# anneouyang/OuterSPACE

Hardware: AMD Instinct MI355X
Metric: spgemm_output_nnz_per_s (higher is better)
Workload: dtype f64

## Files before the change

### outerspace_amd/csrc/osp_api.hip

```cpp
#include <hip/hip_runtime.h>

#include <algorithm>
#include <cmath>
#include <cstdarg>
#include <cstdio>
#include <cstdlib>
#include <chrono>
#include <cstring>
#include <functional>
#include <limits>
#include <map>
#include <memory>
#include <string>
#include <vector>

#include "../../include/outerspace_spgemm.h"
#include "../../include/outerspace_spgemm_masked.h"
#include "../../include/outerspace_spgemm_mcl.h"
#include "../../include/outerspace_spgemm_apply_mask.h"
#include "../../include/outerspace_spgemm_select.h"
#include "../../include/outerspace_spgemm_ewise.h"
#include "../../include/outerspace_spgemm_vector.h"
#include "../../include/outerspace_spgemm_mxm.h"
#include "../../include/outerspace_spgemm_transpose.h"
// ... 193 lines not shown
    uint64_t P = 0;
    const int algo = cfg.algorithm;
    if (algo != OSP_ALGO_OUTER && algo != OSP_ALGO_ROWWISE) throw Error(OSP_ERR_ARG, "unknown algorithm");
    const bool rowwise = algo == OSP_ALGO_ROWWISE && nnz && (uint64_t)nnz_b < 0xffffffffull && nnz < 0xffffffffull && !partials_only;
    ChunkTable<T> ct{};
    const uint64_t direct_min_nnz = getenv("OSP_DIRECT_MIN_NNZ") ? strtoull(getenv("OSP_DIRECT_MIN_NNZ"), nullptr, 10) : ((getenv("OSP_GATHER") && atoi(getenv("OSP_GATHER")) == 0) ? (8ull << 20) : (2ull << 20));
    const bool dense_avg = (long double)p_all * 8.0L >= 3.0L * (long double)M * (long double)N;
    const bool direct = nnz && (nnz >= direct_min_nnz || dense_avg) && (uint64_t)nnz_b < 0xffffffffull && nnz < 0xffffffffull && !partials_only &&
                        !(getenv("OSP_DIRECT") && atoi(getenv("OSP_DIRECT")) == 0);
    const uint64_t direct_max = std::min<uint64_t>(getenv("OSP_DIRECT_MAX") ? strtoull(getenv("OSP_DIRECT_MAX"), nullptr, 10) : kSplitRowMax,
                                                   kDirectDenseMax);
    const int gather_env = getenv("OSP_GATHER") ? atoi(getenv("OSP_GATHER")) : 2;
    const bool gather_ok = nnz && !rowwise && !partials_only && (uint64_t)nnz_b < 0xffffffffull && nnz < 0xffffffffull;
    const bool gather_short = gather_ok && gather_env >= 2 && direct;
    ShortRuns<T> srun{};
    DirectSrc dsrc{};
    uint32_t n_long_rows = 1;
    if (nnz == 0) {
        OSP_HIP(hipMemsetAsync(row_off, 0, (M + 1) * sizeof(uint64_t), s));
    } else {
        Scratch ss(ctx);
        Scratch &keep = (rowwise || direct || gather_short) ? sc : ss;
        const RowSort rs(ss, nnz, std::max(1, bits_for(M)));
        uint32_t *rows_sorted = (gather_short ? keep : ss).template get<uint32_t>(nnz), *perm = keep.get<uint32_t>(nnz), *w_sorted = ss.get<uint32_t>(nnz);
        uint32_t *bs_sorted = (rowwise || direct || gather_short) ? keep.get<uint32_t>(nnz) : nullptr;
        uint32_t *rowfirst = keep.get<uint32_t>(M + 1);
        uint64_t *offs_sorted = keep.get<uint64_t>(nnz + 1);
        uint64_t *scan_tmp = ss.get<uint64_t>(scan_scratch_entries(std::max<uint64_t>(nnz, M + 1)));
        const bool table = rowwise || direct || gather_short;
        const bool with_av = gather_ok && gather_env >= 1 && (direct || gather_short);
        T *av_sorted = with_av ? keep.get<T>(nnz) : nullptr;
        uint32_t *w = ss.get<uint32_t>(with_av ? 4 * nnz : table ? 2 * nnz : nnz);
        uint32_t *bs = table ? w : nullptr;
        sym_chunk_len_kernel<<<grid_for(nnz, 256), 256, 0, s>>>(a_colptr, b_rowptr, k0, k1, e0, nnz, w, bs,
                                                                with_av ? reinterpret_cast<const uint32_t *>(a_vals) : nullptr, (uint32_t)(sizeof(T) / 4));
        SymEpilogue sym_ep{w, bs, rows_sorted, perm, w_sorted, bs_sorted};
        if (with_av) { sym_ep.av_sorted = av_sorted; sym_ep.vwords = (uint32_t)(sizeof(T) / 4); }
        rs.sort(a_rowidx + e0, sym_ep);
        device_exclusive_scan<LoadU32As64, uint64_t>(LoadU32As64{w_sorted}, nnz, offs_sorted, scan_tmp, s);
        sym_row_offsets_kernel<<<grid_for(M + 1, 256), 256, 0, s>>>(rows_sorted, offs_sorted, nnz, M, row_off, rowfirst);
        const uint64_t rw_cap = (rowwise || gather_short) ? (uint64_t)TileCap<T>::value : 0ull;
        const bool expand_rows_on = gather_short && !(getenv("OSP_EXPAND_ROWS") && atoi(getenv("OSP_EXPAND_ROWS")) == 0);
        if (!expand_rows_on) sym_scatter_offsets_kernel<<<grid_for(nnz, 256), 256, 0, s>>>(perm, offs_sorted, rows_sorted, row_off, rw_cap, nnz, chunk_off);
        if (partials_only || rowwise || row_sharded) P = d2h(offs_sorted + nnz, s);
        else P = kPartialsOnDevice;
        if (direct) {
            dsrc = DirectSrc{rowfirst, offs_sorted, bs_sorted, perm, b_colidx, chunk_off, direct_max};
            dsrc.b_rowptr = b_rowptr; dsrc.K = K; dsrc.nnz_b = (uint64_t)nnz_b; dsrc.keep = &sc;
            dsrc.gather = gather_ok && gather_env >= 1;
            dsrc.expand_rows = expand_rows_on;
            if (expand_rows_on) { dsrc.chunk_off_ready = false; dsrc.rows_sorted = rows_sorted; dsrc.row_off = row_off; dsrc.rw_cap = rw_cap; dsrc.nnz = nnz; }
            dsrc.a_vals = with_av ? (const void *)av_sorted : (const void *)(a_vals + e0); dsrc.av_in_order = with_av; dsrc.b_vals = b_vals;
            if (dsrc.gather) {
                dsrc.gstat = (unsigned long long *)sc.get<uint64_t>(3);
                zero_async(s, {{dsrc.gstat, 3 * sizeof(uint64_t)}});
            }
        }
        if (gather_short) {
            const ShortRunFlag sf{offs_sorted};
            uint32_t *cidx = ss.get<uint32_t>(nnz + 1), *cidx_tmp = ss.get<uint32_t>(scan_scratch_entries(nnz + 1));
            device_exclusive_scan<ShortRunFlag, uint32_t>(sf, nnz, cidx, cidx_tmp, s);
            RunDesc<T> *runs0 = sc.get<RunDesc<T>>(nnz);
            uint32_t *rowfirst0 = sc.get<uint32_t>(M + 1);
            short_runs_kernel<T><<<grid_for(nnz, 256), 256, 0, s>>>(sf, cidx, nnz, bs_sorted, av_sorted, runs0);
            short_rowfirst_kernel<<<grid_for(M + 1, 256), 256, 0, s>>>(rowfirst, cidx, M, rowfirst0);
            srun = ShortRuns<T>{runs0, rowfirst0, b_colidx, b_vals};
        }
        if (rowwise) {
            ct = ChunkTable<T>{offs_sorted, bs_sorted, perm, rowfirst, a_vals + e0, b_colidx, b_vals, (uint32_t)rw_cap, 1u};
            uint32_t *flag_scan = ss.get<uint32_t>(M + 1);
            device_exclusive_scan<HeavyRowFlag, uint32_t>(HeavyRowFlag{row_off, 0, (uint32_t)rw_cap}, M, flag_scan, (uint32_t *)scan_tmp, s);
            n_long_rows = d2h(flag_scan + M, s);
        }
    }
    tm.end(PH_SYM);
    res->info.partials = P;

    OuterProducer<T> prod;
    prod.ctx = ctx; prod.res = res;
    prod.a_colptr = a_colptr; prod.a_rowidx = a_rowidx; prod.a_vals = a_vals;
    prod.b_rowptr = b_rowptr; prod.b_colidx = b_colidx; prod.b_vals = b_vals;
    prod.k0 = k0; prod.k1 = k1; prod.e0 = e0; prod.chunk_off = chunk_off;
    const uint64_t nk = k1 - k0;
    prod.a_start = sc.get<int64_t>(nk); prod.a_cnt = sc.get<uint32_t>(nk);
    prod.prod = sc.get<uint64_t>(nk); prod.prod_off = sc.get<uint64_t>(nk + 1);
    prod.scan_tmp = sc.get<uint64_t>(scan_scratch_entries(nk));
    prod.nothing_staged = rowwise && n_long_rows == 0;
    prod.short_gathered = gather_short;
    if ((dsrc.gather || gather_short) && nnz && !partials_only) {
        prod.nnz = nnz;
        prod.kscan = sc.get<uint32_t>(nnz + 1);
        prod.kscan_tmp = sc.get<uint32_t>(scan_scratch_entries(std::max<uint64_t>(nnz, k1 - k0) + 1));
        prod.elist = sc.get<uint32_t>(nnz);
        prod.cscan = sc.get<uint32_t>(k1 - k0 + 1);
        prod.klist = sc.get<uint32_t>(k1 - k0 + 1);
    }

    if (partials_only) {
        if (row_sharded) throw Error(OSP_ERR_ARG, "partial products of a row shard are not supported");
        res->partials = true;
        res->rowptr = (int64_t *)ctx->alloc((M + 1) * sizeof(int64_t));
        OSP_HIP(hipMemcpyAsync(res->rowptr, row_off, (M + 1) * sizeof(uint64_t), hipMemcpyDeviceToDevice, s));
        res->vals = ctx->alloc(std::max<uint64_t>(P, 1) * sizeof(Part<T>));
        res->info.panels = 1;
        res->info.nnz_c = P;
        res->info.row_begin = 0;
        res->info.row_end = M;
        tm.begin(PH_MUL);
        if (P) prod.produce(0, M, true, 0, P, (Part<T> *)res->vals, tm, nullptr, nullptr);
        tm.end(PH_MUL);
        finish_timing(res, ev, tm, s);
        return;
    }
    const uint64_t off_lo = 0, P_rows = P;
    merge_pipeline<T>(ctx, res, prod, M, N, row_off, P_rows, cfg.partial_capacity, tm, r_lo, r_hi, off_lo, sink,
                      rowwise ? &ct : nullptr, (direct && nnz) ? &dsrc : nullptr, nullptr, gather_short ? &srun : nullptr);

    finish_timing(res, ev, tm, s);
    if (gather_short) res->info.gathered_short_partials = res->info.partials - res->info.heavy_partials;
    if (dsrc.gstat && res->info.direct_rows) {
        uint64_t gs[3] = {0, 0, 0};
        copy_d2h(gs, dsrc.gstat, sizeof(gs), s);
        res->info.gathered_rows = gs[0]; res->info.gathered_partials = gs[1]; res->info.gathered_runs = gs[2];
    }
    if (getenv("OSP_VERBOSE")) {
        fprintf(stderr, "[osp] product done in %.1f ms; pool misses so far: %llu hipMalloc calls, %.1f GB, %.1f ms\n", res->info.ms_total,
                (unsigned long long)ctx->malloc_calls, ctx->malloc_bytes / 1e9, ctx->malloc_ms);
    }
}

template <class T>
static void coo_to_compressed_device(Context *ctx, Scratch &sc, uint64_t nseg, uint64_t ninner, uint64_t nnz, const uint32_t *seg,
                                     const uint32_t *inner, const T *vals, const char *what, int64_t **ptr_out,
                                     uint32_t **idx_out, T **val_out) {
    hipStream_t s = ctx->stream;
    int64_t *ptr = sc.get<int64_t>(nseg + 1);
    uint32_t *idx = sc.get<uint32_t>(nnz);
    T *ov = sc.get<T>(nnz);
    *ptr_out = ptr; *idx_out = idx; *val_out = ov;
    if (nnz == 0) {
        OSP_HIP(hipMemsetAsync(ptr, 0, (nseg + 1) * sizeof(int64_t), s));
        return;
    }
    Scratch ss(ctx);
    uint32_t *flags = ss.get<uint32_t>(1);
    OSP_HIP(hipMemsetAsync(flags, 0, sizeof(uint32_t), s));
    const CooOrder o = coo_sort_two_keys(ss, nnz, inner, std::max(1, bits_for(ninner)), seg, std::max(1, bits_for(nseg)));
    ingest_finish_kernel<T><<<grid_for(nnz, 256), 256, 0, s>>>(o.outer_sorted, o.perm, inner, vals, nnz, nseg, ninner, idx, ov, flags);
    ingest_ptr_kernel<<<grid_for(nseg + 1, 256), 256, 0, s>>>(o.outer_sorted, nnz, nseg, ptr);
    check_flags(d2h(flags, s), what);
}

template <class T>
static void spgemm_coo_impl(Context *ctx, Result *res, uint64_t M, uint64_t K, uint64_t N, uint64_t nnz_a, const uint32_t *a_rows,
                            const uint32_t *a_cols, const T *a_vals, uint64_t nnz_b, const uint32_t *b_rows, const uint32_t *b_cols,
                            const T *b_vals, osp_memspace_t space, const osp_config_t &cfg) {
    hipStream_t s = ctx->stream;
    Scratch sc(ctx);
    EventPair ev;
    OSP_HIP(hipEventRecord(ev.a, s));
    const uint32_t *ar = to_device(sc, a_rows, nnz_a, space, s), *ac = to_device(sc, a_cols, nnz_a, space, s);
    const uint32_t *br = to_device(sc, b_rows, nnz_b, space, s), *bc = to_device(sc, b_cols, nnz_b, space, s);
    const T *av = to_device(sc, a_vals, nnz_a, space, s), *bv = to_device(sc, b_vals, nnz_b, space, s);
    int64_t *ap, *bp;
    uint32_t *ai, *bi;
    T *acv, *bcv;
    coo_to_compressed_device<T>(ctx, sc, K, M, nnz_a, ac, ar, av, "A (COO)", &ap, &ai, &acv);
    coo_to_compressed_device<T>(ctx, sc, K, N, nnz_b, br, bc, bv, "B (COO)", &bp, &bi, &bcv);
    OSP_HIP(hipEventRecord(ev.b, s));
    osp_config_t c2 = cfg;
    c2.validate = 0;
    spgemm_impl<T>(ctx, res, M, K, N, ap, ai, acv, bp, bi, bcv, OSP_DEVICE, c2);
    const float ms = ev.ms();
    res->info.ms_ingest = ms;
    res->info.ms_total += ms;
}
// ... 993 lines not shown
```

### outerspace_amd/csrc/osp_pipeline.h

```cpp
#pragma once

#define OSP_WITH_RA(ctx_, ...)                                               \
    do {                                                                     \
        if ((ctx_)->rank_atomic) { constexpr bool RA = true; __VA_ARGS__; }  \
        else { constexpr bool RA = false; __VA_ARGS__; }                     \
    } while (0)

template <class T> struct Producer {
    virtual ~Producer() {}
    virtual void produce(uint64_t r0, uint64_t r1, bool whole, uint64_t base, uint64_t count,
                         Part<T> *stage, PhaseTimer &tm, const uint32_t *cells = nullptr, Part<T> *qstage = nullptr,
                         const HubArgs *hub = nullptr, bool compact = false, bool has_long = true, bool desc_only = false, bool walk_all = false) = 0;
};

template <class T> struct MergeIO {
    Part<T> *stage;
    const uint64_t *row_off; uint64_t r0, r1, base;
    int64_t *c_rowptr; uint32_t *c_col; T *c_val;
    const uint64_t *out_in; uint64_t *out_out;
    ChunkTable<T> ct{};
    uint32_t *abort_word = nullptr;
    const RunDesc<T> *runs0 = nullptr; const uint32_t *rowfirst0 = nullptr; const uint32_t *b_colidx = nullptr; const T *b_vals = nullptr;
};
template <class T> struct ShortRuns {
// ... 164 lines not shown
        device_exclusive_scan<LoadU64, uint64_t>(LoadU64{nhist}, nlong, pl.hbase, pl.hscan_tmp, s);
        if (ds) device_exclusive_scan<LoadU64, uint64_t>(LoadU64{ncellh}, nlong, pl.cellbase, pl.hscan_tmp, s);
        if (ds && nrund) device_exclusive_scan<LoadU64, uint64_t>(LoadU64{nrund}, nlong, rdbase, pl.hscan_tmp, s);
        ndcell = 0;
        nrd = 0;
        {
            Gather g(s);
            g.add(&pl.nh, (const uint64_t *)pl.hoff + nlong); g.add(&pl.nblocks, (const uint64_t *)pl.blkbase + nlong);
            g.add(&pl.nvirt, (const uint64_t *)pl.vbase + nlong); g.add(&pl.ncell, (const uint64_t *)pl.hbase + nlong);
            if (ds) g.add(&ndcell, (const uint64_t *)pl.cellbase + nlong);
            if (ds && nrund) g.add(&nrd, (const uint64_t *)rdbase + nlong);
            for (int i = 0; i < 6; i++) g.add(&tot[i], (const uint64_t *)totals + i);
            g.add(&nsmall, (const uint64_t *)totals + 6);
            g.wait();
        }
        if (ds && ndcell >= 0xffffffffull) { ds = nullptr; hub_b = 0; continue; }
        if (hub_possible && !hub_decided && hub_b == 0 && pl.nblocks && (double)tot[3 + kModeStretch] >= hub_min_share * (double)count) {
            hub_decided = true;
            hub_b = hub_b_want;
            continue;
        }
        break;
    }
    for (int m = 0; m < 3; m++) { pl.mode_rows[m] = tot[m]; pl.mode_partials[m] = tot[3 + m]; }
    if (pl.nh >= 0xffffffffull) throw Error(OSP_ERR_CAPACITY, "long rows of one panel exceed 2^32 partial products");
    res->info.heavy_rows += nlong;
    res->info.heavy_partials += pl.nh;
    res->info.direct_rows += pl.mode_rows[kModeDirect];
    res->info.direct_partials += pl.mode_partials[kModeDirect];
    if (pl.ncell >= 0xffffffffull || pl.nblocks >= 0x7fffffffull || pl.nvirt >= 0xffffffffull || ndcell >= 0xffffffffull)
        throw Error(OSP_ERR_CAPACITY, "split histogram too large");
    if (getenv("OSP_VERBOSE"))
        fprintf(stderr, "[osp]   panel rows [%llu,%llu): %u tiles, %u long rows with %llu partial products -> %llu segments; direct: %llu rows, %llu "
                        "partial products, %llu cells\n",
                (unsigned long long)r0, (unsigned long long)r1, pl.p0.ntiles, nlong, (unsigned long long)pl.nh, (unsigned long long)pl.nvirt,
                (unsigned long long)pl.mode_rows[kModeDirect], (unsigned long long)pl.mode_partials[kModeDirect], (unsigned long long)ndcell);
    pl.ghist = sc.get<uint32_t>(pl.ncell + 1);
    pl.ghist_tmp = sc.get<uint32_t>(scan_scratch_entries(pl.ncell + 1));
    pl.vrow_off = sc.get<uint64_t>(pl.nvirt + 1);
    pl.vfirst = sc.get<uint8_t>(pl.nvirt + 1);
    pl.vcol0 = sc.get<uint32_t>(pl.nvirt + 1);
    pl.vcol1 = sc.get<uint32_t>(pl.nvirt + 1);
    if (pl.mode_rows[kModeDirect]) {
        pl.cells = sc.get<uint32_t>(ndcell);
        GatherPlan gp{};
        RunDesc<T> *runs = nullptr;
        static const uint64_t max_runs = getenv("OSP_GATHER_MAX_RUNS") ? strtoull(getenv("OSP_GATHER_MAX_RUNS"), nullptr, 10) : 0xffffffffull;
        if (ds->gather && nrund && nrd < max_runs) {
            runs = sc.get<RunDesc<T>>(std::max<uint64_t>(nrd, 1));
            pl.vrun_off = sc.get<uint32_t>(pl.nvirt + 1);
            pl.vrun_end = sc.get<uint32_t>(pl.nvirt + 1);
            gp.rdbase = rdbase; gp.vrun_off = pl.vrun_off; gp.vrun_end = pl.vrun_end;
            gp.rowruns = sc.get<uint32_t>(nlong);
            pl.nwritten = gp.nwritten = sc.get<uint32_t>(1);
            fill_async(s, {{pl.vrun_off, (pl.nvirt + 1) * sizeof(uint32_t), kNoRuns}, {gp.rowruns, (uint64_t)nlong * sizeof(uint32_t), kNoRuns},
                           {pl.nwritten, sizeof(uint32_t), 0u}});
            gp.over = !(getenv("OSP_GATHER_OVER") && atoi(getenv("OSP_GATHER_OVER")) == 0);
            gp.av_in_order = ds->av_in_order ? 1u : 0u;
            pl.may_write = !gp.over;
            pl.ga.runs = runs; pl.ga.b_colidx = ds->b_colidx; pl.ga.b_vals = (const T *)ds->b_vals;
        }
        if (!(runs && gp.over) || (hub_b && pl.nblocks)) ds->ensure_chunk_off(s);
        gp.mark_skipped = ds->chunk_off_ready ? 1u : 0u;
        const bool plan_small = runs != nullptr && gp.over && nsmall != 0;
        const bool plan_big = !plan_small || nsmall < pl.mode_rows[kModeDirect];
        if (plan_small) gp.small = hsmall;
        if (getenv("OSP_VERBOSE"))
            fprintf(stderr, "[osp]   small planner: %llu of %llu direct rows (at most %u chunks, %u cells)\n", (unsigned long long)(plan_small ? nsmall : 0),
                    (unsigned long long)pl.mode_rows[kModeDirect], small_lim.chunks, small_lim.cells);
        tm.begin(PH_PLAN_K, s);
        if (plan_small)
            direct_plan_small_kernel<T><<<nlong, kWave, direct_plan_small_lds(small_lim.cells), s>>>(
                pl.p0.long_rows, nlong, pl.hbits, nseg, pl.vbase, pl.hoff, colbits, kCap, ds->rowfirst, ds->off, ds->bs, ds->perm, ds->b_colidx,
                pl.vrow_off, pl.vcol0, pl.vcol1, ds->chunk_off, gp, (const T *)ds->a_vals, runs);
        if (!plan_big) {  }
        else if (nlong <= 4u * ctx->cus)
            direct_plan_kernel<T, kDirectCellsBig><<<nlong, kDirectThreads, 0, s>>>(pl.p0.long_rows, nlong, pl.hmode, pl.hbits, nseg, pl.vbase, pl.hoff,
                                                                                 pl.cellbase, row_off, colbits, kCap, ds->rowfirst, ds->off, ds->bs, ds->perm,
                                                                                 ds->b_colidx, pl.vrow_off, pl.vcol0, pl.vcol1, pl.cells, ds->chunk_off, gp,
                                                                                 (const T *)ds->a_vals, runs);
        else
        direct_plan_kernel<T><<<nlong, kDirectThreads, 0, s>>>(pl.p0.long_rows, nlong, pl.hmode, pl.hbits, nseg, pl.vbase, pl.hoff, pl.cellbase, row_off,
                                                              colbits, kCap, ds->rowfirst, ds->off, ds->bs, ds->perm, ds->b_colidx, pl.vrow_off,
                                                              pl.vcol0, pl.vcol1, pl.cells, ds->chunk_off, gp, (const T *)ds->a_vals, runs);
        tm.end(PH_PLAN_K);
        if (gp.rowruns && ds->gstat) gather_stats_kernel<<<std::min(grid_for(nlong, 256), 64u), 256, 0, s>>>(pl.p0.long_rows, nlong, row_off, gp.rowruns, ds->gstat);
#ifdef OSP_PLAN_PROF
        if (getenv("OSP_VERBOSE")) {
            unsigned long long hp[8] = {0}, z[8] = {0};
            OSP_HIP(hipStreamSynchronize(s));
            (void)hipMemcpyFromSymbol(hp, HIP_SYMBOL(osp_plan_prof), sizeof(hp));
            (void)hipMemcpyToSymbol(HIP_SYMBOL(osp_plan_prof), z, sizeof(z));
            double tot = 0;
            for (int k = 0; k < 6; k++) tot += (double)hp[k];
            fprintf(stderr, "[osp]   planner cycles: header %.1f %%, chunk descriptors %.1f %%, histogram pass %.1f %%, grouping %.1f %%, cell pass %.1f %%, "
                            "prefixes + output %.1f %%; %.0f cycles per row, %u rows\n", 100 * hp[0] / tot, 100 * hp[1] / tot, 100 * hp[2] / tot, 100 * hp[3] / tot,
                    100 * hp[4] / tot, 100 * hp[5] / tot, tot / std::max(1u, nlong), nlong);
            (void)hipMemcpyFromSymbol(hp, HIP_SYMBOL(osp_plan_small_prof), sizeof(hp));
            (void)hipMemcpyToSymbol(HIP_SYMBOL(osp_plan_small_prof), z, sizeof(z));
            tot = 0;
            for (int k = 0; k < 5; k++) tot += (double)hp[k];
            if (plan_small && tot > 0)
                fprintf(stderr, "[osp]   small planner cycles: header + chunk descriptors %.1f %%, histogram pass %.1f %%, grouping %.1f %%, counts %.1f %%, "
                                "prefixes + output %.1f %%; %.0f cycles per row, %llu rows\n", 100 * hp[0] / tot, 100 * hp[1] / tot, 100 * hp[2] / tot,
                        100 * hp[3] / tot, 100 * hp[4] / tot, tot / (double)nsmall, (unsigned long long)nsmall);
        }
#endif
        res->info.direct_plan_launches++;
        dbg_sync(s, "plan of the direct rows");
    }
    if (hub_b && pl.nblocks) {
        if (!ds->hub.sx) {
            Scratch &keep = *ds->keep;
            const uint64_t nb = ds->nnz_b;
            Scratch tmp(ctx);
            uint8_t *rowstart = tmp.get<uint8_t>(nb + 4);
            uint32_t *sx = keep.get<uint32_t>(nb + 1), *runstart = keep.get<uint32_t>(nb + 1);
            uint16_t *runblk = keep.get<uint16_t>(nb + 2);
            uint32_t *scan_tmp = tmp.get<uint32_t>(scan_scratch_entries(nb + 1));
            OSP_HIP(hipMemsetAsync(rowstart, 0, nb + 4, s));
            hub_rowstart_kernel<<<grid_for(ds->K, 256), 256, 0, s>>>(ds->b_rowptr, ds->K, rowstart);
            const int sh = colbits - hub_b;
            const HubRunFlag flag{rowstart, ds->b_colidx, sh};
            device_exclusive_scan<HubRunFlag, uint32_t>(flag, nb, sx, scan_tmp, s);
            compact_flagged_kernel<HubRunFlag><<<grid_for(nb, 256), 256, 0, s>>>(flag, sx, nb, 0, runstart);
            hub_runstart_end_kernel<<<1, 1, 0, s>>>(sx + nb, runstart, (uint32_t)nb);
            OSP_HIP(hipMemsetAsync(runblk, 0, (nb + 2) * sizeof(uint16_t), s));
            hub_runblk_kernel<<<std::min(grid_for(nb, 256), 4096u), 256, 0, s>>>(sx + nb, runstart, ds->b_colidx, sh, runblk);
            OSP_HIP(hipStreamSynchronize(s));
            ds->hub.sx = sx; ds->hub.runstart = runstart; ds->hub.runblk = runblk; ds->hub.sh = sh;
        }
        tm.begin(PH_HUB_K, s);
        uint64_t *jobruns = sc.get<uint64_t>(pl.nblocks + 1);
        uint64_t *jobscan_tmp = sc.get<uint64_t>(scan_scratch_entries(pl.nblocks + 1));
        const size_t hub_lds = sizeof(uint32_t) << hub_b;
        hub_plan_kernel<false><<<(unsigned)pl.nblocks, kHubThreads, hub_lds, s>>>(pl.p0.long_rows, nlong, pl.blkbase, pl.hbase, pl.hbits, pl.nstretch, row_off,
                                                                           ds->rowfirst, ds->off, ds->bs, ds->perm, ds->b_colidx, ds->hub, pl.ghist,
                                                                           pl.hoff, jobruns, nullptr, nullptr, nullptr);
        device_exclusive_scan<LoadU32, uint32_t>(LoadU32{pl.ghist}, pl.ncell, pl.ghist, pl.ghist_tmp, s);
// ... 660 lines not shown
```

### outerspace_amd/csrc/osp_split.h

```cpp
#pragma once
#include "osp_kernels.h"

namespace osp {

#ifndef OSP_SPLIT_THREADS
#define OSP_SPLIT_THREADS 256
#endif
constexpr int kSplitThreads = OSP_SPLIT_THREADS;
#ifndef OSP_SPLIT_ROW_THREADS
#define OSP_SPLIT_ROW_THREADS 1024
#endif
#ifndef OSP_SPLIT_ROW_PRE
#define OSP_SPLIT_ROW_PRE 1
#endif
constexpr int kSplitRowThreads = OSP_SPLIT_ROW_THREADS;
#ifndef OSP_SPLIT_ROW_STRETCH
#define OSP_SPLIT_ROW_STRETCH 4096
#endif
constexpr int kSplitRowStretch = OSP_SPLIT_ROW_STRETCH;
#ifndef OSP_SPLIT_STRETCH
#define OSP_SPLIT_STRETCH 4096
#endif
constexpr int kSplitStretch = OSP_SPLIT_STRETCH;
#ifndef OSP_SPLIT_JOB_ROUNDS
// ... 505 lines not shown
        __syncthreads();
        for (uint32_t d = threadIdx.x; d < nseg; d += kSplitRowThreads) segoff[d] += cnt[NW][d];
    }
}
__device__ __forceinline__ uint64_t lanes_above_mask() { return lane_id() == 63 ? 0ull : (~0ull << (lane_id() + 1)); }
__device__ __forceinline__ bool wave_run_head(uint32_t key, bool valid, uint32_t &runlen, uint64_t above) {
    const unsigned lane = lane_id();
    const uint32_t prev = wave_shr1(key);
    const bool head = valid && (lane == 0 || key != prev);
    const uint64_t heads = __builtin_amdgcn_ballot_w64(head), vm = __builtin_amdgcn_ballot_w64(valid);
    const uint64_t rest = heads & above;
    const uint32_t next = rest ? (uint32_t)__builtin_ctzll(rest) : (uint32_t)__popcll(vm);
    runlen = next - lane;
    return head;
}
#ifndef OSP_DIRECT_UNR
#define OSP_DIRECT_UNR 8
#endif
#ifndef OSP_PLAN_RUNS
#define OSP_PLAN_RUNS 1
#endif
#ifndef OSP_DIRECT_CHUNK_BLOCK
#define OSP_DIRECT_CHUNK_BLOCK 512
#endif
#ifndef OSP_DIRECT_CELLS_LDS
#define OSP_DIRECT_CELLS_LDS 1024
#endif
constexpr int kDirectChunkBlock = OSP_DIRECT_CHUNK_BLOCK;
__device__ __forceinline__ uint32_t direct_find_chunk(const uint32_t *cst, uint32_t n, uint32_t i) {
    uint32_t lo = 0, hi = n;
    while (hi - lo > 1) { const uint32_t mid = (lo + hi) >> 1; if (cst[mid] <= i) lo = mid; else hi = mid; }
    return lo;
}
#ifdef OSP_PLAN_PROF
__device__ unsigned long long osp_plan_prof[8];
#define OSP_PLAN_MARK(k) do { if (threadIdx.x == 0) { const unsigned long long now_ = clock64(); atomicAdd(&osp_plan_prof[k], now_ - prof_t); prof_t = now_; } } while (0)
#define OSP_PLAN_DECL unsigned long long prof_t = clock64();
__device__ unsigned long long osp_plan_small_prof[8];
#define OSP_PLAN_SMALL_MARK(k) do { if (threadIdx.x == 0) { const unsigned long long now_ = clock64(); atomicAdd(&osp_plan_small_prof[k], now_ - prof_t); prof_t = now_; } } while (0)
#else
#define OSP_PLAN_MARK(k)
#define OSP_PLAN_SMALL_MARK(k)
#define OSP_PLAN_DECL
#endif
struct GatherPlan {
    const uint64_t *rdbase = nullptr;
    uint32_t *vrun_off = nullptr, *vrun_end = nullptr;
    uint32_t *rowruns = nullptr;
    uint32_t *nwritten = nullptr;
    uint32_t over = 1;
    uint32_t mark_skipped = 1;
    uint32_t av_in_order = 0;
    const uint8_t *small = nullptr;
};
__global__ void gather_stats_kernel(const uint32_t *rows, uint32_t nlong, const uint64_t *row_off, const uint32_t *rowruns, unsigned long long *gstat) {
    uint64_t nr = 0, np = 0, nd = 0;
    for (uint32_t h = blockIdx.x * blockDim.x + threadIdx.x; h < nlong; h += gridDim.x * blockDim.x) {
        const uint32_t r = rowruns[h];
        if (r != kNoRuns) { nr++; nd += r; np += row_off[rows[h] + 1] - row_off[rows[h]]; }
    }
    nr = wave_reduce_sum<uint64_t>(nr); np = wave_reduce_sum<uint64_t>(np); nd = wave_reduce_sum<uint64_t>(nd);
    if (lane_id() == 0 && nr) { atomicAdd(&gstat[0], (unsigned long long)nr); atomicAdd(&gstat[1], (unsigned long long)np); atomicAdd(&gstat[2], (unsigned long long)nd); }
}
constexpr int kDirectCellsBig = 8 * OSP_DIRECT_CELLS_LDS;
template <class V, int CL = OSP_DIRECT_CELLS_LDS>
__global__ __launch_bounds__(kDirectThreads, (CL > OSP_DIRECT_CELLS_LDS ? 2 : 8)) void direct_plan_kernel(
    const uint32_t *__restrict__ rows, uint32_t nlong, const uint8_t *__restrict__ hmode, const uint8_t *__restrict__ hbits,
    const uint32_t *__restrict__ nseg, const uint64_t *__restrict__ vbase, const uint64_t *__restrict__ hoff,
    const uint64_t *__restrict__ cellbase, const uint64_t *__restrict__ row_off, int colbits, uint32_t cap,
    const uint32_t *__restrict__ rowfirst, const uint64_t *__restrict__ ct_off, const uint32_t *__restrict__ ct_bs,
    const uint32_t *__restrict__ perm, const uint32_t *__restrict__ b_colidx, uint64_t *__restrict__ vrow_off,
    uint32_t *__restrict__ vcol0, uint32_t *__restrict__ vcol1, uint32_t *__restrict__ cells, uint64_t *__restrict__ chunk_off,
    const GatherPlan gp, const V *__restrict__ a_vals, RunDesc<V> *__restrict__ runs) {
    constexpr int NT = kDirectThreads, NFINE = 1 << kDirectFineBits, CBL = kDirectChunkBlock, UNR = OSP_DIRECT_UNR;
    constexpr int kCellsLds = CL;
    constexpr bool kBigCells = CL > OSP_DIRECT_CELLS_LDS;
    __shared__ V avs_own[kBigCells ? CBL : 1];
    __shared__ alignas(8) uint32_t hist[NFINE + 1];
    __shared__ alignas(4) uint16_t nxt[NFINE];
    __shared__ uint8_t lut[NFINE];
    __shared__ uint32_t rbin0[kDirectMaxRanges + 2], roff[kDirectMaxRanges + 2], cursor[kDirectMaxRanges + 1];
    __shared__ uint32_t cbs[CBL], cst[CBL + 1];
    __shared__ uint32_t cellm[kCellsLds], lsm[kCellsLds];
    __shared__ uint32_t psum[NT];
    __shared__ uint32_t scratch[NT / kWave + 1];
    __shared__ uint32_t s_T, s_over;
    const uint32_t h = blockIdx.x;
    if (h >= nlong || hmode[h] != kModeDirect) return;
    if (gp.small != nullptr && gp.small[h]) return;
    OSP_PLAN_DECL
    const unsigned tid = threadIdx.x, lane = lane_id(), w = tid >> 6;
    const uint64_t above = lanes_above_mask();
    const uint32_t i = rows[h];
    const uint32_t c0 = rowfirst[i], nc = rowfirst[i + 1] - c0;
    const uint32_t b = hbits[h], nfine = 1u << b, Ta = nseg[h];
    const int sh = colbits - (int)b;
    const uint32_t q0 = (uint32_t)hoff[h];
    uint32_t *__restrict__ rb = cells + cellbase[h];
    const uint32_t lutw = (nfine + 3) / 4;
    auto load_block = [&](uint32_t cb, uint32_t nb) {
        uint32_t len[CBL / NT], bsv[CBL / NT], sum = 0;
#pragma unroll
        for (int q = 0; q < CBL / NT; q++) {
            const uint32_t j = tid * (CBL / NT) + q;
            len[q] = 0; bsv[q] = 0;
            if (j < nb) {
                const uint32_t c = c0 + cb + j;
                bsv[q] = ct_bs[c];
                len[q] = (uint32_t)(ct_off[c + 1] - ct_off[c]);
            }
            sum += len[q];
        }
        uint32_t total;
        uint32_t ex = block_excl_scan<uint32_t, NT>(sum, scratch, &total);
#pragma unroll
        for (int q = 0; q < CBL / NT; q++) {
            const uint32_t j = tid * (CBL / NT) + q;
            if (j < nb) { cst[j] = ex; cbs[j] = bsv[q] - ex; }
            ex += len[q];
        }
        if (tid == 0) cst[nb] = total;
        __syncthreads();
        return total;
    };
    auto for_entries = [&](uint32_t nb, uint32_t E, auto f) {
        for (uint32_t base = w * (UNR * kWave); base < E; base += NT * UNR) {
            uint32_t cu[UNR], col[UNR];
            uint32_t c = direct_find_chunk(cst, nb, base);
#pragma unroll
            for (int u = 0; u < UNR; u++) {
                const uint32_t e = base + u * kWave + lane;
                const bool valid = e < E;
                while (valid && e >= cst[c + 1]) c++;
                cu[u] = c;
                col[u] = b_colidx[valid ? cbs[c] + e : 0u];
            }
#pragma unroll
            for (int u = 0; u < UNR; u++) f(cu[u], col[u], base + u * kWave + lane < E);
        }
    };
    for (uint32_t d = tid; d <= nfine; d += NT) hist[d] = 0;
    __syncthreads();
    OSP_PLAN_MARK(0);
    uint32_t have_cb = 0, have_nb = 0, have_E = 0;
    for (uint32_t cb = 0; cb < nc; cb += CBL) {
        const uint32_t nb = min((uint32_t)CBL, nc - cb);
        const uint32_t E = load_block(cb, nb);
        OSP_PLAN_MARK(1);
        have_cb = cb; have_nb = nb; have_E = E;
        for_entries(nb, E, [&](uint32_t, uint32_t col, bool valid) {
#if OSP_PLAN_RUNS
            const uint32_t bin = valid ? col >> sh : 0xffffffffu;
            uint32_t runlen;
            if (wave_run_head(bin, valid, runlen, above)) atomicAdd(&hist[bin], runlen);
#else
            if (valid) atomicAdd(&hist[col >> sh], 1u);
#endif
        });
        __syncthreads();
        OSP_PLAN_MARK(2);
    }
    {
        constexpr int PER = NFINE / NT;
        static_assert(NFINE % NT == 0 && PER >= 1, "the fine bins are scanned PER per thread");
        uint32_t v[PER], sum = 0;
#pragma unroll
        for (int q = 0; q < PER; q++) { const uint32_t d = tid * PER + q; v[q] = d < nfine ? hist[d] : 0u; sum += v[q]; }
        uint32_t total;
        uint32_t ex = block_excl_scan<uint32_t, NT>(sum, scratch, &total);
#pragma unroll
        for (int q = 0; q < PER; q++) { const uint32_t d = tid * PER + q; if (d < nfine) hist[d] = ex; ex += v[q]; }
        if (tid == 0) hist[nfine] = total;
    }
    __syncthreads();
    for (uint32_t d = tid; d < nfine; d += NT) {
        const uint32_t lim = hist[d] + cap;
        uint32_t lo = d + 1, hi = nfine + 1;
        while (lo < hi) { const uint32_t mid = (lo + hi) >> 1; if (hist[mid] <= lim) lo = mid + 1; else hi = mid; }
        nxt[d] = (uint16_t)max(d + 1, lo - 1);
    }
    __syncthreads();
    if (tid == 0) {
        uint32_t t = 0, over = 0;
        for (uint32_t d = 0; d < nfine; d = nxt[d]) { rbin0[t] = d; roff[t] = hist[d]; over |= (hist[nxt[d]] - hist[d]) > cap ? 1u : 0u; t++; }
        rbin0[t] = nfine; roff[t] = hist[nfine];
        s_T = t;
        s_over = over;
    }
    __syncthreads();
    const uint32_t T = s_T;
    const bool gathered = gp.rdbase != nullptr && (s_over == 0 || gp.over);
    for (uint32_t d = tid; d < nfine; d += NT) {
        uint32_t lo = 0, hi = T;
        while (hi - lo > 1) { const uint32_t mid = (lo + hi) >> 1; if (rbin0[mid] <= d) lo = mid; else hi = mid; }
        lut[d] = (uint8_t)lo;
    }
    for (uint32_t t = tid; t < Ta; t += NT) {
        const uint64_t v = vbase[h] + t;
        const uint32_t tt = min(t, T);
        vrow_off[v] = (uint64_t)q0 + roff[tt];
        vcol0[v] = (uint32_t)min((uint64_t)rbin0[tt] << sh, (uint64_t)0xffffffffu);
        vcol1[v] = (uint32_t)min((uint64_t)rbin0[min(tt + 1, T)] << sh, (uint64_t)0xffffffffu);
        if (t < T) cursor[t] = 0;
    }
    __syncthreads();
    if (gathered) {
        constexpr uint32_t kAvMax = kBigCells ? (uint32_t)CBL : (uint32_t)((NFINE + 1) * sizeof(uint32_t) / (sizeof(V)));
        const uint32_t CB = max(1u, min(min((uint32_t)CBL, (uint32_t)kCellsLds / T), kAvMax));
        const bool multi = nc > CB;
        V *avs = kBigCells ? avs_own : reinterpret_cast<V *>(hist);
        uint32_t *nzc = reinterpret_cast<uint32_t *>(nxt), *ncur = rbin0;
        static_assert(sizeof(nxt) >= (kDirectMaxRanges + 1) * sizeof(uint32_t), "runs per range: where the grouping's chain was");
        const uint32_t rowbase = (uint32_t)gp.rdbase[h];
        static_assert(kDirectMaxRanges + 1 <= NT, "one range per thread");
        const uint32_t bcol_t = tid <= T ? (uint32_t)min((uint64_t)rbin0[tid] << sh, (uint64_t)0xffffffffu) : 0u;
        __syncthreads();
        if (tid <= T) { nzc[tid] = 0; ncur[tid] = 0; if (tid < T) cursor[tid] = bcol_t; }
        if (!multi) { for (uint32_t cl = tid; cl < nc; cl += NT) avs[cl] = gp.av_in_order ? a_vals[c0 + cl] : a_vals[perm[c0 + cl]]; }
        __syncthreads();
        for (uint32_t cb = 0; cb < nc; cb += CB) {
            const uint32_t nb = min(CB, nc - cb);
            for (uint32_t x = tid; x < nb * T; x += NT) cellm[x] = 0;
            uint32_t E = have_E;
            if (cb != have_cb || nb != have_nb) E = load_block(cb, nb);
            else __syncthreads();
            have_cb = cb; have_nb = nb; have_E = E;
            OSP_PLAN_MARK(1);
            if (T > 1 && (uint64_t)E >= (uint64_t)nb * (T - 1) * 8u) {
                for (uint32_t x = tid; x < nb * (T - 1); x += NT) {
                    const uint32_t cl = x / (T - 1), t = x - cl * (T - 1) + 1;
                    const uint32_t col = cursor[t], b0 = cbs[cl] + cst[cl];
                    uint32_t lo = 0, hi = cst[cl + 1] - cst[cl];
                    while (lo < hi) { const uint32_t mid = (lo + hi) >> 1; if (b_colidx[b0 + mid] < col) lo = mid + 1; else hi = mid; }
                    lsm[cl * T + t] = lo;
                }
                for (uint32_t cl = tid; cl < nb; cl += NT) lsm[cl * T] = 0;
                __syncthreads();
                for (uint32_t x = tid; x < nb * T; x += NT) {
                    const uint32_t cl = x / T, t = x - cl * T;
                    cellm[x] = (t + 1 < T ? lsm[x + 1] : cst[cl + 1] - cst[cl]) - lsm[x];
                }
            } else {
                for_entries(nb, E, [&](uint32_t cl, uint32_t col, bool valid) {
                    const uint32_t key = valid ? __umul24(cl, T) + (uint32_t)lut[col >> sh] : 0xffffffffu;
                    uint32_t runlen;
                    if (wave_run_head(key, valid, runlen, above)) atomicAdd(&cellm[key], runlen);
                });
            }
            __syncthreads();
            OSP_PLAN_MARK(4);
            for (uint32_t x = tid; x < nb * T; x += NT) {
                const uint32_t c = cellm[x], cl = x / T, t = x - cl * T;
                if (c) atomicAdd(&nzc[t], 1u);
                if (multi) rb[lutw + (uint64_t)(cb + cl) * Ta + t] = c;
            }
            __syncthreads();
        }
        {
            const uint32_t v = tid < T ? nzc[tid] : 0u;
            uint32_t total;
            const uint32_t ex = block_excl_scan<uint32_t, NT>(v, scratch, &total);
            if (tid < T) nzc[tid] = ex;
            if (tid == 0) {
                nzc[T] = total;
                gp.rowruns[h] = total;
            }
            if (tid < T) cursor[tid] = 0;
        }
        __syncthreads();
        for (uint32_t t = tid; t < Ta; t += NT) {
            const uint64_t v = vbase[h] + t;
            gp.vrun_off[v] = rowbase + nzc[min(t, T)];
            gp.vrun_end[v] = rowbase + nzc[min(t + 1, T)];
        }
        const uint32_t G = max(1u, min((uint32_t)NT / T, 16u));
        for (uint32_t cb = 0; cb < nc; cb += CB) {
            const uint32_t nb = min(CB, nc - cb);
            if (multi) {
                if (cb != have_cb || nb != have_nb) { have_E = load_block(cb, nb); have_cb = cb; have_nb = nb; }
                for (uint32_t x = tid; x < nb * T; x += NT) { const uint32_t cl = x / T, t = x - cl * T; cellm[x] = rb[lutw + (uint64_t)(cb + cl) * Ta + t]; }
            }
            if (multi) { for (uint32_t cl = tid; cl < nb; cl += NT) avs[cl] = gp.av_in_order ? a_vals[c0 + cb + cl] : a_vals[perm[c0 + cb + cl]]; }
            __syncthreads();
            for (uint32_t cl = tid; cl < nb; cl += NT) {
                uint32_t run = 0;
                for (uint32_t t = 0; t < T; t++) { lsm[cl * T + t] = run; run += cellm[cl * T + t]; }
            }
            const uint32_t S = (nb + G - 1) / G;
            for (uint32_t t0 = 0; t0 < T; t0 += NT) {
                const uint32_t Tb = min((uint32_t)NT, T - t0);
                const uint32_t g = tid / Tb, t = t0 + (tid - g * Tb);
                const bool on = g < G;
                uint32_t run0 = 0, nrun0 = 0;
                __syncthreads();
                if (on) {
                    uint32_t sum = 0, nz = 0;
                    static_assert(kDirectDenseMax <= (1ull << 20) && CBL < 2048, "products and runs of a group of chunks in one word");
                    for (uint32_t cl = g * S; cl < min(nb, (g + 1) * S); cl++) { const uint32_t c = cellm[cl * T + t]; sum += c; nz += c != 0; }
                    psum[tid] = sum | (nz << 21);
                    run0 = cursor[t];
                    nrun0 = ncur[t];
                }
                __syncthreads();
                if (on) {
                    uint32_t run = run0, nrun = nrun0;
                    for (uint32_t gg = 0; gg < g; gg++) { const uint32_t p = psum[gg * Tb + (t - t0)]; run += p & 0x1fffffu; nrun += p >> 21; }
                    const uint32_t rbase = q0 + roff[t];
                    RunDesc<V> *__restrict__ out = runs + rowbase + nzc[t];
                    for (uint32_t cl = g * S; cl < min(nb, (g + 1) * S); cl++) {
                        const uint32_t c = cellm[cl * T + t];
                        if (c) {
                            RunDesc<V> rd;
                            rd.dst = rbase + run;
                            rd.src = cbs[cl] + cst[cl] + lsm[cl * T + t];
                            rd.av = avs[cl];
                            out[nrun++] = rd;
                        }
                        run += c;
                    }
                    if (g == G - 1) { cursor[t] = run; ncur[t] = nrun; }
                }
            }
            if (gp.mark_skipped) { for (uint32_t cl = tid; cl < nb; cl += NT) chunk_off[perm[c0 + cb + cl]] = kChunkSkip; }
            __syncthreads();
            OSP_PLAN_MARK(5);
        }
        return;
    }
    for (uint32_t d = tid; d < lutw * 4; d += NT) reinterpret_cast<uint8_t *>(rb)[d] = d < nfine ? lut[d] : (uint8_t)0;
    if (tid == 0 && gp.rdbase != nullptr && gp.nwritten) atomicAdd(gp.nwritten, 1u);
    OSP_PLAN_MARK(3);
    const uint32_t CB = max(1u, min((uint32_t)CBL, (uint32_t)kCellsLds / T));
    const uint32_t G = max(1u, min((uint32_t)NT / T, 16u));
    for (uint32_t cb = 0; cb < nc; cb += CB) {
        const uint32_t nb = min(CB, nc - cb);
        for (uint32_t x = tid; x < nb * T; x += NT) cellm[x] = 0;
        uint32_t E = have_E;
        if (cb != have_cb || nb != have_nb) E = load_block(cb, nb);
        else __syncthreads();
        have_cb = cb; have_nb = nb; have_E = E;
        OSP_PLAN_MARK(1);
        for_entries(nb, E, [&](uint32_t cl, uint32_t col, bool valid) {
#if OSP_PLAN_RUNS
            const uint32_t key = valid ? __umul24(cl, T) + (uint32_t)lut[col >> sh] : 0xffffffffu;
            uint32_t runlen;
            if (wave_run_head(key, valid, runlen, above)) atomicAdd(&cellm[key], runlen);
#else
            if (valid) atomicAdd(&cellm[__umul24(cl, T) + (uint32_t)lut[col >> sh]], 1u);
#endif
        });
        __syncthreads();
        OSP_PLAN_MARK(4);
        for (uint32_t cl = tid; cl < nb; cl += NT) {
            uint32_t run = 0;
            for (uint32_t t = 0; t < T; t++) { lsm[cl * T + t] = run; run += cellm[cl * T + t]; }
        }
        const uint32_t S = (nb + G - 1) / G;
        for (uint32_t t0 = 0; t0 < T; t0 += NT) {
            const uint32_t Tb = min((uint32_t)NT, T - t0);
            const uint32_t g = tid / Tb, t = t0 + (tid - g * Tb);
            const bool on = g < G;
            uint32_t run0 = 0;
            __syncthreads();
            if (on) {
                uint32_t sum = 0;
                for (uint32_t cl = g * S; cl < min(nb, (g + 1) * S); cl++) sum += cellm[cl * T + t];
                psum[tid] = sum;
                run0 = cursor[t];
            }
            __syncthreads();
            if (on) {
                uint32_t run = run0;
                for (uint32_t gg = 0; gg < g; gg++) run += psum[gg * Tb + (t - t0)];
                const uint32_t rbase = q0 + roff[t];
                for (uint32_t cl = g * S; cl < min(nb, (g + 1) * S); cl++) {
                    rb[lutw + (uint64_t)(cb + cl) * Ta + t] = rbase + run - lsm[cl * T + t];
                    run += cellm[cl * T + t];
                }
                if (g == G - 1) cursor[t] = run;
// ... 295 lines not shown
```

Measured before the change: 69.80 billion.

## Restructure gathered planner into descriptor blocks with fused prefix-offset cell storage

The gathered-row planner now loads chunk descriptors in CBL-sized blocks and walks them in reverse during the counting phase, so the last loaded block is reused by the emission phase. Cells are stored once as exclusive prefix offsets with a trailing total (stride T+1) in a merged LDS array, which replaces the separate count and prefix arrays and roughly doubles how many chunks fit per sub-block. The intent is to cut repeated descriptor loads and barriers. In exchange it adds per-row block counters and extra statistics written to global memory, plus more index arithmetic.

```diff
diff --git a/outerspace_amd/csrc/osp_api.hip b/outerspace_amd/csrc/osp_api.hip
--- a/outerspace_amd/csrc/osp_api.hip
+++ b/outerspace_amd/csrc/osp_api.hip
@@ -269,8 +269,8 @@
             if (expand_rows_on) { dsrc.chunk_off_ready = false; dsrc.rows_sorted = rows_sorted; dsrc.row_off = row_off; dsrc.rw_cap = rw_cap; dsrc.nnz = nnz; }
             dsrc.a_vals = with_av ? (const void *)av_sorted : (const void *)(a_vals + e0); dsrc.av_in_order = with_av; dsrc.b_vals = b_vals;
             if (dsrc.gather) {
-                dsrc.gstat = (unsigned long long *)sc.get<uint64_t>(3);
-                zero_async(s, {{dsrc.gstat, 3 * sizeof(uint64_t)}});
+                dsrc.gstat = (unsigned long long *)sc.get<uint64_t>(kGatherStats);
+                zero_async(s, {{dsrc.gstat, kGatherStats * sizeof(uint64_t)}});
             }
         }
         if (gather_short) {
@@ -336,9 +336,11 @@
     finish_timing(res, ev, tm, s);
     if (gather_short) res->info.gathered_short_partials = res->info.partials - res->info.heavy_partials;
     if (dsrc.gstat && res->info.direct_rows) {
-        uint64_t gs[3] = {0, 0, 0};
+        uint64_t gs[kGatherStats] = {0, 0, 0, 0, 0};
         copy_d2h(gs, dsrc.gstat, sizeof(gs), s);
         res->info.gathered_rows = gs[0]; res->info.gathered_partials = gs[1]; res->info.gathered_runs = gs[2];
+        if (getenv("OSP_VERBOSE"))
+            fprintf(stderr, "[osp] planner blocks: %llu descriptor loads, %llu blocks of cells per phase\n", (unsigned long long)gs[3], (unsigned long long)gs[4]);
     }
     if (getenv("OSP_VERBOSE")) {
         fprintf(stderr, "[osp] product done in %.1f ms; pool misses so far: %llu hipMalloc calls, %.1f GB, %.1f ms\n", res->info.ms_total,
diff --git a/outerspace_amd/csrc/osp_pipeline.h b/outerspace_amd/csrc/osp_pipeline.h
--- a/outerspace_amd/csrc/osp_pipeline.h
+++ b/outerspace_amd/csrc/osp_pipeline.h
@@ -240,9 +240,11 @@
             pl.vrun_end = sc.get<uint32_t>(pl.nvirt + 1);
             gp.rdbase = rdbase; gp.vrun_off = pl.vrun_off; gp.vrun_end = pl.vrun_end;
             gp.rowruns = sc.get<uint32_t>(nlong);
+            gp.rowblocks = sc.get<uint32_t>(2 * (uint64_t)nlong);
             pl.nwritten = gp.nwritten = sc.get<uint32_t>(1);
             fill_async(s, {{pl.vrun_off, (pl.nvirt + 1) * sizeof(uint32_t), kNoRuns}, {gp.rowruns, (uint64_t)nlong * sizeof(uint32_t), kNoRuns},
-                           {pl.nwritten, sizeof(uint32_t), 0u}});
+                           {pl.nwritten, sizeof(uint32_t), 0u}, {gp.rowblocks, 2 * (uint64_t)nlong * sizeof(uint32_t), 0u}});
+            gp.blocks = (uint32_t)std::clamp(getenv("OSP_PLAN_BLOCKS") ? atoi(getenv("OSP_PLAN_BLOCKS")) : 2, 0, 2);
             gp.over = !(getenv("OSP_GATHER_OVER") && atoi(getenv("OSP_GATHER_OVER")) == 0);
             gp.av_in_order = ds->av_in_order ? 1u : 0u;
             pl.may_write = !gp.over;
@@ -272,7 +274,7 @@
                                                               colbits, kCap, ds->rowfirst, ds->off, ds->bs, ds->perm, ds->b_colidx, pl.vrow_off,
                                                               pl.vcol0, pl.vcol1, pl.cells, ds->chunk_off, gp, (const T *)ds->a_vals, runs);
         tm.end(PH_PLAN_K);
-        if (gp.rowruns && ds->gstat) gather_stats_kernel<<<std::min(grid_for(nlong, 256), 64u), 256, 0, s>>>(pl.p0.long_rows, nlong, row_off, gp.rowruns, ds->gstat);
+        if (gp.rowruns && ds->gstat) gather_stats_kernel<<<std::min(grid_for(nlong, 256), 64u), 256, 0, s>>>(pl.p0.long_rows, nlong, row_off, gp.rowruns, ds->gstat, gp.rowblocks);
 #ifdef OSP_PLAN_PROF
         if (getenv("OSP_VERBOSE")) {
             unsigned long long hp[8] = {0}, z[8] = {0};
diff --git a/outerspace_amd/csrc/osp_split.h b/outerspace_amd/csrc/osp_split.h
--- a/outerspace_amd/csrc/osp_split.h
+++ b/outerspace_amd/csrc/osp_split.h
@@ -581,15 +581,22 @@
     uint32_t mark_skipped = 1;
     uint32_t av_in_order = 0;
     const uint8_t *small = nullptr;
+    uint32_t blocks = 1;
+    uint32_t *rowblocks = nullptr;
 };
-__global__ void gather_stats_kernel(const uint32_t *rows, uint32_t nlong, const uint64_t *row_off, const uint32_t *rowruns, unsigned long long *gstat) {
-    uint64_t nr = 0, np = 0, nd = 0;
+constexpr int kGatherStats = 5;
+__global__ void gather_stats_kernel(const uint32_t *rows, uint32_t nlong, const uint64_t *row_off, const uint32_t *rowruns, unsigned long long *gstat,
+                                    const uint32_t *rowblocks) {
+    uint64_t nr = 0, np = 0, nd = 0, nl = 0, nb = 0;
     for (uint32_t h = blockIdx.x * blockDim.x + threadIdx.x; h < nlong; h += gridDim.x * blockDim.x) {
         const uint32_t r = rowruns[h];
         if (r != kNoRuns) { nr++; nd += r; np += row_off[rows[h] + 1] - row_off[rows[h]]; }
+        if (rowblocks) { nl += rowblocks[2 * h]; nb += rowblocks[2 * h + 1]; }
     }
     nr = wave_reduce_sum<uint64_t>(nr); np = wave_reduce_sum<uint64_t>(np); nd = wave_reduce_sum<uint64_t>(nd);
+    nl = wave_reduce_sum<uint64_t>(nl); nb = wave_reduce_sum<uint64_t>(nb);
     if (lane_id() == 0 && nr) { atomicAdd(&gstat[0], (unsigned long long)nr); atomicAdd(&gstat[1], (unsigned long long)np); atomicAdd(&gstat[2], (unsigned long long)nd); }
+    if (lane_id() == 0 && nb) { atomicAdd(&gstat[3], (unsigned long long)nl); atomicAdd(&gstat[4], (unsigned long long)nb); }
 }
 constexpr int kDirectCellsBig = 8 * OSP_DIRECT_CELLS_LDS;
 template <class V, int CL = OSP_DIRECT_CELLS_LDS>
@@ -610,7 +617,8 @@
     __shared__ uint8_t lut[NFINE];
     __shared__ uint32_t rbin0[kDirectMaxRanges + 2], roff[kDirectMaxRanges + 2], cursor[kDirectMaxRanges + 1];
     __shared__ uint32_t cbs[CBL], cst[CBL + 1];
-    __shared__ uint32_t cellm[kCellsLds], lsm[kCellsLds];
+    __shared__ uint32_t cells_lds[2 * kCellsLds];
+    uint32_t *const cellm = cells_lds, *const lsm = cells_lds + kCellsLds;
     __shared__ uint32_t psum[NT];
     __shared__ uint32_t scratch[NT / kWave + 1];
     __shared__ uint32_t s_T, s_over;
@@ -652,22 +660,24 @@
         __syncthreads();
         return total;
     };
-    auto for_entries = [&](uint32_t nb, uint32_t E, auto f) {
-        for (uint32_t base = w * (UNR * kWave); base < E; base += NT * UNR) {
+    auto for_entries_at = [&](uint32_t sb, uint32_t nb, uint32_t e0, uint32_t e1, auto f) {
+        const uint32_t *cs = cst + sb, *bs = cbs + sb;
+        for (uint32_t base = e0 + w * (UNR * kWave); base < e1; base += NT * UNR) {
             uint32_t cu[UNR], col[UNR];
-            uint32_t c = direct_find_chunk(cst, nb, base);
+            uint32_t c = direct_find_chunk(cs, nb, base);
 #pragma unroll
             for (int u = 0; u < UNR; u++) {
                 const uint32_t e = base + u * kWave + lane;
-                const bool valid = e < E;
-                while (valid && e >= cst[c + 1]) c++;
+                const bool valid = e < e1;
+                while (valid && e >= cs[c + 1]) c++;
                 cu[u] = c;
-                col[u] = b_colidx[valid ? cbs[c] + e : 0u];
-            }
-#pragma unroll
-            for (int u = 0; u < UNR; u++) f(cu[u], col[u], base + u * kWave + lane < E);
+                col[u] = b_colidx[valid ? bs[c] + e : 0u];
+            }
+#pragma unroll
+            for (int u = 0; u < UNR; u++) f(cu[u], col[u], base + u * kWave + lane < e1);
         }
     };
+    auto for_entries = [&](uint32_t nb, uint32_t E, auto f) { for_entries_at(0u, nb, 0u, E, f); };
     for (uint32_t d = tid; d <= nfine; d += NT) hist[d] = 0;
     __syncthreads();
     OSP_PLAN_MARK(0);
@@ -735,8 +745,10 @@
     __syncthreads();
     if (gathered) {
         constexpr uint32_t kAvMax = kBigCells ? (uint32_t)CBL : (uint32_t)((NFINE + 1) * sizeof(uint32_t) / (sizeof(V)));
-        const uint32_t CB = max(1u, min(min((uint32_t)CBL, (uint32_t)kCellsLds / T), kAvMax));
+        const uint32_t T1 = T + 1;
+        const uint32_t CB = max(1u, min(min((uint32_t)CBL, gp.blocks >= 2 ? 2u * (uint32_t)kCellsLds / T1 : (uint32_t)kCellsLds / T), kAvMax));
         const bool multi = nc > CB;
+        uint32_t *const st = cells_lds;
         V *avs = kBigCells ? avs_own : reinterpret_cast<V *>(hist);
         uint32_t *nzc = reinterpret_cast<uint32_t *>(nxt), *ncur = rbin0;
         static_assert(sizeof(nxt) >= (kDirectMaxRanges + 1) * sizeof(uint32_t), "runs per range: where the grouping's chain was");
@@ -747,43 +759,51 @@
         if (tid <= T) { nzc[tid] = 0; ncur[tid] = 0; if (tid < T) cursor[tid] = bcol_t; }
         if (!multi) { for (uint32_t cl = tid; cl < nc; cl += NT) avs[cl] = gp.av_in_order ? a_vals[c0 + cl] : a_vals[perm[c0 + cl]]; }
         __syncthreads();
-        for (uint32_t cb = 0; cb < nc; cb += CB) {
-            const uint32_t nb = min(CB, nc - cb);
-            for (uint32_t x = tid; x < nb * T; x += NT) cellm[x] = 0;
-            uint32_t E = have_E;
-            if (cb != have_cb || nb != have_nb) E = load_block(cb, nb);
-            else __syncthreads();
-            have_cb = cb; have_nb = nb; have_E = E;
-            OSP_PLAN_MARK(1);
-            if (T > 1 && (uint64_t)E >= (uint64_t)nb * (T - 1) * 8u) {
-                for (uint32_t x = tid; x < nb * (T - 1); x += NT) {
-                    const uint32_t cl = x / (T - 1), t = x - cl * (T - 1) + 1;
-                    const uint32_t col = cursor[t], b0 = cbs[cl] + cst[cl];
-                    uint32_t lo = 0, hi = cst[cl + 1] - cst[cl];
-                    while (lo < hi) { const uint32_t mid = (lo + hi) >> 1; if (b_colidx[b0 + mid] < col) lo = mid + 1; else hi = mid; }
-                    lsm[cl * T + t] = lo;
+        const uint32_t D = gp.blocks ? (uint32_t)CBL : CB, nD = (nc + D - 1) / D;
+        uint32_t nload = 0, nsub = 0;
+        for (uint32_t di = 0; di < nD; di++) {
+            const uint32_t db = (gp.blocks ? nD - 1 - di : di) * D, nd = min(D, nc - db);
+            const bool load = db != have_cb || nd != have_nb;
+            for (uint32_t sb = 0; sb < nd; sb += CB) {
+                const uint32_t nb = min(CB, nd - sb), cb = db + sb;
+                if (load && sb == 0) { have_E = load_block(db, nd); have_cb = db; have_nb = nd; nload++; }
+                nsub++;
+                const uint32_t *scst = cst + sb, *scbs = cbs + sb;
+                const uint32_t e0 = scst[0], e1 = scst[nb], E = e1 - e0;
+                OSP_PLAN_MARK(1);
+                if (T > 1 && (uint64_t)E >= (uint64_t)nb * (T - 1) * 8u) {
+                    for (uint32_t x = tid; x < nb * (T - 1); x += NT) {
+                        const uint32_t cl = x / (T - 1), t = x - cl * (T - 1) + 1;
+                        const uint32_t col = cursor[t], b0 = scbs[cl] + scst[cl];
+                        uint32_t lo = 0, hi = scst[cl + 1] - scst[cl];
+                        while (lo < hi) { const uint32_t mid = (lo + hi) >> 1; if (b_colidx[b0 + mid] < col) lo = mid + 1; else hi = mid; }
+                        st[cl * T1 + t] = lo;
+                    }
+                    for (uint32_t cl = tid; cl < nb; cl += NT) { st[cl * T1] = 0; st[cl * T1 + T] = scst[cl + 1] - scst[cl]; }
+                } else {
+                    for (uint32_t x = tid; x < nb * T1; x += NT) st[x] = 0;
+                    __syncthreads();
+                    for_entries_at(sb, nb, e0, e1, [&](uint32_t cl, uint32_t col, bool valid) {
+                        const uint32_t key = valid ? __umul24(cl, T1) + (uint32_t)lut[col >> sh] : 0xffffffffu;
+                        uint32_t runlen;
+                        if (wave_run_head(key, valid, runlen, above)) atomicAdd(&st[key], runlen);
+                    });
+                    __syncthreads();
+                    for (uint32_t cl = tid; cl < nb; cl += NT) {
+                        uint32_t run = 0;
+                        for (uint32_t t = 0; t < T; t++) { const uint32_t c = st[cl * T1 + t]; st[cl * T1 + t] = run; run += c; }
+                        st[cl * T1 + T] = run;
+                    }
                 }
-                for (uint32_t cl = tid; cl < nb; cl += NT) lsm[cl * T] = 0;
                 __syncthreads();
+                OSP_PLAN_MARK(4);
                 for (uint32_t x = tid; x < nb * T; x += NT) {
-                    const uint32_t cl = x / T, t = x - cl * T;
-                    cellm[x] = (t + 1 < T ? lsm[x + 1] : cst[cl + 1] - cst[cl]) - lsm[x];
+                    const uint32_t cl = x / T, t = x - cl * T, s0 = st[x + cl];
+                    if (st[x + cl + 1] != s0) atomicAdd(&nzc[t], 1u);
+                    if (multi) rb[lutw + (uint64_t)(cb + cl) * Ta + t] = s0;
                 }
-            } else {
-                for_entries(nb, E, [&](uint32_t cl, uint32_t col, bool valid) {
-                    const uint32_t key = valid ? __umul24(cl, T) + (uint32_t)lut[col >> sh] : 0xffffffffu;
-                    uint32_t runlen;
-                    if (wave_run_head(key, valid, runlen, above)) atomicAdd(&cellm[key], runlen);
-                });
-            }
-            __syncthreads();
-            OSP_PLAN_MARK(4);
-            for (uint32_t x = tid; x < nb * T; x += NT) {
-                const uint32_t c = cellm[x], cl = x / T, t = x - cl * T;
-                if (c) atomicAdd(&nzc[t], 1u);
-                if (multi) rb[lutw + (uint64_t)(cb + cl) * Ta + t] = c;
-            }
-            __syncthreads();
+                __syncthreads();
+            }
         }
         {
             const uint32_t v = tid < T ? nzc[tid] : 0u;
@@ -803,57 +823,59 @@
             gp.vrun_end[v] = rowbase + nzc[min(t + 1, T)];
         }
         const uint32_t G = max(1u, min((uint32_t)NT / T, 16u));
-        for (uint32_t cb = 0; cb < nc; cb += CB) {
-            const uint32_t nb = min(CB, nc - cb);
-            if (multi) {
-                if (cb != have_cb || nb != have_nb) { have_E = load_block(cb, nb); have_cb = cb; have_nb = nb; }
-                for (uint32_t x = tid; x < nb * T; x += NT) { const uint32_t cl = x / T, t = x - cl * T; cellm[x] = rb[lutw + (uint64_t)(cb + cl) * Ta + t]; }
-            }
-            if (multi) { for (uint32_t cl = tid; cl < nb; cl += NT) avs[cl] = gp.av_in_order ? a_vals[c0 + cb + cl] : a_vals[perm[c0 + cb + cl]]; }
-            __syncthreads();
-            for (uint32_t cl = tid; cl < nb; cl += NT) {
-                uint32_t run = 0;
-                for (uint32_t t = 0; t < T; t++) { lsm[cl * T + t] = run; run += cellm[cl * T + t]; }
-            }
-            const uint32_t S = (nb + G - 1) / G;
-            for (uint32_t t0 = 0; t0 < T; t0 += NT) {
-                const uint32_t Tb = min((uint32_t)NT, T - t0);
-                const uint32_t g = tid / Tb, t = t0 + (tid - g * Tb);
-                const bool on = g < G;
-                uint32_t run0 = 0, nrun0 = 0;
+        for (uint32_t di = 0; di < nD; di++) {
+            const uint32_t db = di * D, nd = min(D, nc - db);
+            const bool load = multi && (db != have_cb || nd != have_nb);
+            for (uint32_t sb = 0; sb < nd; sb += CB) {
+                const uint32_t nb = min(CB, nd - sb), cb = db + sb;
+                const uint32_t *scst = cst + sb, *scbs = cbs + sb;
+                if (multi) {
+                    if (load && sb == 0) { have_E = load_block(db, nd); have_cb = db; have_nb = nd; nload++; }
+                    for (uint32_t x = tid; x < nb * T; x += NT) { const uint32_t cl = x / T, t = x - cl * T; st[x + cl] = rb[lutw + (uint64_t)(cb + cl) * Ta + t]; }
+                    for (uint32_t cl = tid; cl < nb; cl += NT) st[cl * T1 + T] = scst[cl + 1] - scst[cl];
+                }
+                if (multi) { for (uint32_t cl = tid; cl < nb; cl += NT) avs[cl] = gp.av_in_order ? a_vals[c0 + cb + cl] : a_vals[perm[c0 + cb + cl]]; }
+                const uint32_t S = (nb + G - 1) / G;
+                for (uint32_t t0 = 0; t0 < T; t0 += NT) {
+                    const uint32_t Tb = min((uint32_t)NT, T - t0);
+                    const uint32_t g = tid / Tb, t = t0 + (tid - g * Tb);
+                    const bool on = g < G;
+                    uint32_t run0 = 0, nrun0 = 0;
+                    __syncthreads();
+                    if (on) {
+                        uint32_t sum = 0, nz = 0;
+                        static_assert(kDirectDenseMax <= (1ull << 20) && CBL < 2048, "products and runs of a group of chunks in one word");
+                        for (uint32_t cl = g * S; cl < min(nb, (g + 1) * S); cl++) { const uint32_t c = st[cl * T1 + t + 1] - st[cl * T1 + t]; sum += c; nz += c != 0; }
+                        psum[tid] = sum | (nz << 21);
+                        run0 = cursor[t];
+                        nrun0 = ncur[t];
+                    }
+                    __syncthreads();
+                    if (on) {
+                        uint32_t run = run0, nrun = nrun0;
+                        for (uint32_t gg = 0; gg < g; gg++) { const uint32_t p = psum[gg * Tb + (t - t0)]; run += p & 0x1fffffu; nrun += p >> 21; }
+                        const uint32_t rbase = q0 + roff[t];
+                        RunDesc<V> *__restrict__ out = runs + rowbase + nzc[t];
+                        for (uint32_t cl = g * S; cl < min(nb, (g + 1) * S); cl++) {
+                            const uint32_t s0 = st[cl * T1 + t], c = st[cl * T1 + t + 1] - s0;
+                            if (c) {
+                                RunDesc<V> rd;
+                                rd.dst = rbase + run;
+                                rd.src = scbs[cl] + scst[cl] + s0;
+                                rd.av = avs[cl];
+                                out[nrun++] = rd;
+                            }
+                            run += c;
+                        }
+                        if (g == G - 1) { cursor[t] = run; ncur[t] = nrun; }
+                    }
+                }
+                if (gp.mark_skipped) { for (uint32_t cl = tid; cl < nb; cl += NT) chunk_off[perm[c0 + cb + cl]] = kChunkSkip; }
                 __syncthreads();
-                if (on) {
-                    uint32_t sum = 0, nz = 0;
-                    static_assert(kDirectDenseMax <= (1ull << 20) && CBL < 2048, "products and runs of a group of chunks in one word");
-                    for (uint32_t cl = g * S; cl < min(nb, (g + 1) * S); cl++) { const uint32_t c = cellm[cl * T + t]; sum += c; nz += c != 0; }
-                    psum[tid] = sum | (nz << 21);
-                    run0 = cursor[t];
-                    nrun0 = ncur[t];
-                }
-                __syncthreads();
-                if (on) {
-                    uint32_t run = run0, nrun = nrun0;
-                    for (uint32_t gg = 0; gg < g; gg++) { const uint32_t p = psum[gg * Tb + (t - t0)]; run += p & 0x1fffffu; nrun += p >> 21; }
-                    const uint32_t rbase = q0 + roff[t];
-                    RunDesc<V> *__restrict__ out = runs + rowbase + nzc[t];
-                    for (uint32_t cl = g * S; cl < min(nb, (g + 1) * S); cl++) {
-                        const uint32_t c = cellm[cl * T + t];
-                        if (c) {
-                            RunDesc<V> rd;
-                            rd.dst = rbase + run;
-                            rd.src = cbs[cl] + cst[cl] + lsm[cl * T + t];
-                            rd.av = avs[cl];
-                            out[nrun++] = rd;
-                        }
-                        run += c;
-                    }
-                    if (g == G - 1) { cursor[t] = run; ncur[t] = nrun; }
-                }
-            }
-            if (gp.mark_skipped) { for (uint32_t cl = tid; cl < nb; cl += NT) chunk_off[perm[c0 + cb + cl]] = kChunkSkip; }
-            __syncthreads();
-            OSP_PLAN_MARK(5);
-        }
+                OSP_PLAN_MARK(5);
+            }
+        }
+        if (tid == 0 && gp.rowblocks) { gp.rowblocks[2 * h] = nload; gp.rowblocks[2 * h + 1] = nsub; }
         return;
     }
     for (uint32_t d = tid; d < lutw * 4; d += NT) reinterpret_cast<uint8_t *>(rb)[d] = d < nfine ? lut[d] : (uint8_t)0;
```

Result: no change. 70.30 billion (median of 6 runs) (+0.7%).
